# GoekeLab/m6anet

Hardware: AMD Instinct MI355X
Metric: DRACH sites/sec at num_iterations=1000 (higher is better)
Workload: dtype f32

## Files before the change

m6anet_amd/csrc/m6a_api.hip:

```cpp
#include "m6a_ctx.h"

#if !defined(__HIP_DEVICE_COMPILE__)
#ifndef M6A_MT_JUMP_PATH
#error "build with -DM6A_MT_JUMP_PATH=\"<repo>/m6anet_amd/assets/mt19937_jump.bin\" (m6anet_amd/build.py does)"
#endif
asm(".section .rodata\n"
    ".global m6a_mt_jump_blob\n.global m6a_mt_jump_blob_end\n.hidden m6a_mt_jump_blob\n.hidden m6a_mt_jump_blob_end\n.balign 64\n"
    "m6a_mt_jump_blob:\n.incbin \"" M6A_MT_JUMP_PATH "\"\n"
    "m6a_mt_jump_blob_end:\n.byte 0\n.previous\n");
#endif

namespace {

thread_local std::string g_create_error;

std::mutex g_live_mu;
std::vector<m6a_ctx *> g_live;
void join_background_setups()
{
    std::lock_guard<std::mutex> g(g_live_mu);
    for (m6a_ctx *c : g_live)
        if (c->warm.joinable()) c->warm.join();
    g_live.clear();
}
// ... 102 lines not shown
    int64_t start_b = 0;
    for (int64_t b = 0; b < nb; b++) {
        if ((it0 + b + 1) % spb) {
            goff.push_back(std::min((b + 1) * bs, S));
            start_b = b + 1;
        }
    }
    if (start_b < nb) goff.push_back(S);
    return (int64_t)goff.size() - 1;
}

bool base_is_group_start(int64_t base, int64_t bs, int64_t spb)
{
    if (base < 0 || base % bs) return false;
    const int64_t it0 = base / bs;
    return it0 == 0 || (it0 % spb) != 0;
}

int ensure_groups(m6a_ctx *c, int64_t S, int64_t bs, int64_t spb)
{
    const int64_t base = c->job_offset;
    if (c->goff_key.valid && c->goff_key.S == S && c->goff_key.bs == bs && c->goff_key.spb == spb &&
        c->goff_key.base == base) return M6A_OK;
    if (!base_is_group_start(base, bs, spb))
        return fail(c, M6A_EINVAL, "job offset %lld does not start a flush group for batch_size=%lld save_per_batch=%lld",
                    (long long)base, (long long)bs, (long long)spb);
    std::vector<int64_t> g;
    const int64_t G = flush_groups(S, bs, spb, base, g);
    int64_t gmax = 0;
    for (int64_t i = 0; i < G; i++) gmax = std::max(gmax, g[i + 1] - g[i]);
    HIPCHK(c, c->goff.ensure(g.size() * sizeof(int64_t)));
    HIPCHK(c, hipMemcpyAsync(c->goff.p, g.data(), g.size() * sizeof(int64_t), hipMemcpyHostToDevice, c->stream));
    HIPCHK(c, hipStreamSynchronize(c->stream));
    c->goff_key = {S, bs, spb, base, G, gmax, true};
    return M6A_OK;
}

constexpr int kJumpPerRegime = 31, kJumpPolyWords = 312;
constexpr int64_t kXheadWords = 22016;

extern "C" const unsigned char m6a_mt_jump_blob[];
extern "C" const unsigned char m6a_mt_jump_blob_end[];

struct JumpRegime { int64_t G; const uint64_t *polys; };

const JumpRegime *jump_regimes(int *n_out)
// ... 40 lines not shown
    }
    const int n_seg = (int)std::min<int64_t>((len + use->G - 1) / use->G, kJumpPerRegime + 1);
    const size_t poly_bytes = (size_t)kJumpPerRegime * kJumpPolyWords * 8;
    HIPCHK(c, c->mt_scratch.ensure((size_t)kXheadWords * 4 + (size_t)kJumpPerRegime * 1078 * 4 + poly_bytes));
    uint32_t *xhead = (uint32_t *)c->mt_scratch.p, *hist = xhead + kXheadWords;
    uint64_t *d_polys = (uint64_t *)(hist + (size_t)kJumpPerRegime * 1078);
    if (c->mt_polys_G != use->G) {
        HIPCHK(c, hipMemcpyAsync(d_polys, use->polys, poly_bytes, hipMemcpyHostToDevice, c->stream));
        c->mt_polys_G = use->G;
    }
    hipLaunchKernelGGL(mt19937_kernel, dim3(1), dim3(640), 0, c->stream, seed, kXheadWords - 624, raw, (const uint32_t *)nullptr,
                       kXheadWords, xhead, kXheadWords);
    hipLaunchKernelGGL(mt_jump_kernel, dim3(17, (unsigned)(n_seg - 1)), dim3(256), 0, c->stream, (const uint32_t *)xhead,
                       (const uint64_t *)d_polys, hist);
    hipLaunchKernelGGL(mt19937_kernel, dim3((unsigned)n_seg), dim3(640), 0, c->stream, seed, len, raw, (const uint32_t *)hist, use->G,
                       (uint32_t *)nullptr, (int64_t)0);
    HIPCHK(c, hipGetLastError());
    return M6A_OK;
}

int ensure_raw(m6a_ctx *c, uint32_t seed, int64_t len)
{
    if (c->raw_len >= len && c->raw_seed == seed) return M6A_OK;
    if (len > ((int64_t)1 << 31) - 512)
        return fail(c, M6A_ESTREAM, "a flush group would need %lld MT19937 words (cap 2^31); "
                    "reduce batch_size*save_per_batch or num_iterations", (long long)len);
    len = (len + 1023) / 1024 * 1024;
    c->raw_len = 0;
    c->rt.valid = false;
    HIPCHK(c, c->raw.ensure((size_t)len * 4));
    int rc = launch_stream(c, seed, len, (uint32_t *)c->raw.p);
    if (rc) return rc;
    c->raw_seed = seed; c->raw_len = len;
    return M6A_OK;
}

void pairwise_rec(int lo, int n, MeanPlan &p)
{
    if (n <= 128) {
        p.leaf_start.push_back(lo);
        p.merge_after.push_back(0);
        return;
    }
    int n2 = n / 2;
    n2 -= n2 % 8;
    pairwise_rec(lo, n2, p);
// ... 37 lines not shown
    }
    p.reg_ctl.assign((size_t)std::max(1, (T - p.n_rem) / 8), 0u);
    for (int b = 0; b + 1 < L; b++) p.reg_ctl[(size_t)p.leaf_start[b + 1] / 8 - 1] = 1u | ((uint32_t)p.merge_after[b] << 8);
    const int rows = (int)p.row_pass.size();
    p.row_meta.assign((size_t)rows * 4, 0u);
    for (int r = 0; r < rows; r++) {
        uint32_t *m = &p.row_meta[(size_t)r * 4];
        uint64_t live = 0;
        for (int l = 0; l < 64; l++) live |= (uint64_t)(plan_iteration(p, r, l) >= 0) << l;
        m[1] = (uint32_t)live; m[2] = (uint32_t)(live >> 32);
        const int ps = p.row_pass[r];
        if (ps < 0) { m[0] = 1u << 25; continue; }
        if (r + 1 == rows || p.row_pass[r + 1] != ps) {
            const int nl = std::min(8, L - 8 * ps);
            m[0] = (1u << 24) | ((uint32_t)nl << 26) | (ps == P - 1 ? 1u << 30 : 0u);
            for (int bl = 0; bl < nl; bl++) m[3] |= (uint32_t)(p.merge_after[8 * ps + bl] & 15) << (4 * bl);
        }
    }
}

int ensure_mean_plan(m6a_ctx *c, int T)
{
    if (c->plan.T == T && c->plan_dev.p) return M6A_OK;
    build_mean_plan(T, c->plan);
    const MeanPlan &p = c->plan;
    if (p.depth > M6A_MEAN_STACK) return fail(c, M6A_EUNSUPPORTED, "n_iters %d: pairwise-sum tree deeper than %d", T, M6A_MEAN_STACK);
    const size_t b0 = p.leaf_start.size() * 4, b1 = (p.merge_after.size() + 3) / 4 * 4, b2 = std::max<size_t>(p.row_meta.size(), 1) * 4;
    const size_t b3 = p.reg_ctl.size() * 4;
    HIPCHK(c, c->plan_dev.ensure(b0 + b1 + b2 + b3));
    char *d = (char *)c->plan_dev.p;
    HIPCHK(c, hipMemcpyAsync(d, p.leaf_start.data(), b0, hipMemcpyHostToDevice, c->stream));
    HIPCHK(c, hipMemcpyAsync(d + b0, p.merge_after.data(), p.merge_after.size(), hipMemcpyHostToDevice, c->stream));
    if (!p.row_meta.empty())
        HIPCHK(c, hipMemcpyAsync(d + b0 + b1, p.row_meta.data(), p.row_meta.size() * 4, hipMemcpyHostToDevice, c->stream));
    HIPCHK(c, hipMemcpyAsync(d + b0 + b1 + b2, p.reg_ctl.data(), b3, hipMemcpyHostToDevice, c->stream));
    HIPCHK(c, hipStreamSynchronize(c->stream));
    c->plan_off[0] = 0; c->plan_off[1] = b0; c->plan_off[2] = b0 + b1; c->plan_off[3] = b0 + b1 + b2;
    c->tab_key.valid = false;
    return M6A_OK;
}

void plan_args(m6a_ctx *c, PoolArgs &a)
{
    const char *d = (const char *)c->plan_dev.p;
    a.leaf_start = (const int *)(d + c->plan_off[0]);
    a.merge_after = (const uint8_t *)(d + c->plan_off[1]);
// ... 29 lines not shown
    if (n_distinct) *n_distinct = distinct;
    return missing;
}

int ensure_rtab(m6a_ctx *c, uint32_t seed, int T, int K, int64_t gmax, const uint32_t *hist, bool *usable)
{
    *usable = false;
    const int64_t need = stream_need(gmax, T, K);
    int rc = ensure_raw(c, seed, need);
    if (rc) return rc;
    auto &rt = c->rt;
    const int64_t n_blk = c->raw_len / 64;
    if (!(rt.valid && rt.seed == seed && rt.A == (int64_t)T * K && rt.n_blk == n_blk)) {
        rt.valid = false; rt.used = 0;
        for (int n = 0; n <= M6A_RTAB_MAX_N; n++) rt.slot_of_n[n] = -1;
    }
    std::vector<int> todo;
    for (int n = 2; n <= M6A_RTAB_MAX_N; n++)
        if (hist[n] && rt.slot_of_n[n] < 0) todo.push_back(n);
    const int64_t c_stride = n_blk * 64;
    const size_t slot_bytes = (size_t)c_stride * 2 + (size_t)(n_blk + 1) * 4;
    const bool fresh = !rt.valid || rt.n_blk != n_blk;
    const int want = (fresh ? 1 : rt.used) + (int)todo.size();
    if (fresh || want > rt.cap) {
        int new_cap = std::max(want, fresh ? 0 : rt.cap * 2);
        new_cap = std::min(std::max(new_cap, std::max(32, c->rt_presize)), M6A_RTAB_MAX_N + 1);
        size_t free_b = 0, total_b = 0;
        HIPCHK(c, hipMemGetInfo(&free_b, &total_b));
        const size_t held = fresh ? 0 : (size_t)rt.cap * slot_bytes;
        const size_t budget = std::min<size_t>((size_t)16 << 30, (free_b + held) / 2);
        if ((size_t)new_cap * slot_bytes > budget) new_cap = want;
        if ((size_t)new_cap * slot_bytes > budget) return M6A_OK;
        uint16_t *nC = nullptr; uint32_t *nRS = nullptr;
        if (fresh) {
            if (rt.C) (void)hipFree(rt.C);
            if (rt.RS) (void)hipFree(rt.RS);
            rt.C = nullptr; rt.RS = nullptr; rt.cap = 0;
        }
        if (hipMalloc((void **)&nC, (size_t)new_cap * c_stride * 2 + 64) != hipSuccess) { (void)hipGetLastError(); return M6A_OK; }
        if (hipMalloc((void **)&nRS, (size_t)new_cap * (n_blk + 1) * 4) != hipSuccess) { (void)hipGetLastError(); (void)hipFree(nC); return M6A_OK; }
        if (!fresh && rt.used) {
            HIPCHK(c, hipMemcpyAsync(nC, rt.C, (size_t)rt.used * c_stride * 2, hipMemcpyDeviceToDevice, c->stream));
            HIPCHK(c, hipMemcpyAsync(nRS, rt.RS, (size_t)rt.used * (n_blk + 1) * 4, hipMemcpyDeviceToDevice, c->stream));
            HIPCHK(c, hipStreamSynchronize(c->stream));
            c->graveyard.push_back(rt.C); c->graveyard.push_back(rt.RS);
        }
// ... 29 lines not shown
int uniform_slice(m6a_ctx *c, uint32_t seed, int n, int T, int K, int jmax, const uint16_t **C)
{
    *C = nullptr;
    if (n < 2) return M6A_OK;
    std::vector<uint32_t> hist(M6A_HIST_BINS, 0u);
    hist[n] = 1;
    bool usable = false;
    int rc = ensure_rtab(c, seed, T, K, jmax, hist.data(), &usable);
    if (rc) return rc;
    if (!usable) return fail(c, M6A_ENOMEM, "no device memory for the index table of bag size %d", n);
    const int64_t slot = c->rt.slot_of_n[n], A = (int64_t)T * K;
    uint32_t total = 0;
    HIPCHK(c, hipMemcpyAsync(&total, c->rt.RS + slot * (c->rt.n_blk + 1) + c->rt.n_blk, 4, hipMemcpyDeviceToHost, c->stream));
    HIPCHK(c, hipStreamSynchronize(c->stream));
    if ((int64_t)total < A * jmax) return fail(c, M6A_ESTREAM, "MT19937 stream too short for a flush group");
    *C = c->rt.C + slot * c->rt.n_blk * 64;
    return M6A_OK;
}

int ensure_table_reg(m6a_ctx *c, uint32_t seed, int n, int T, int K, int jmax)
{
    auto &k = c->tab_reg_key;
    if (k.valid && k.seed == seed && k.n == n && k.T == T && k.K == K && k.jmax >= jmax) return M6A_OK;
    k.valid = false;
    const size_t per_j = (size_t)(T + 8) * K;
    const size_t bytes = (size_t)jmax * per_j * 2 + 4096;
    HIPCHK(c, c->tab_reg.ensure(bytes));
    HIPCHK(c, hipMemsetAsync(c->tab_reg.p, 0, bytes, c->stream));
    const uint16_t *C = nullptr;
    int rc = uniform_slice(c, seed, n, T, K, jmax, &C);
    if (rc) return rc;
    if (C) {
        const int64_t A = (int64_t)T * K;
        hipLaunchKernelGGL(rtab_to_reg_table_kernel, dim3((unsigned)((A * jmax + 255) / 256)), dim3(256), 0, c->stream,
                           C, A, (int64_t)per_j, jmax, (uint16_t *)c->tab_reg.p);
        HIPCHK(c, hipGetLastError());
    }
    k = {seed, n, T, K, jmax, true};
    return M6A_OK;
}

int ensure_table(m6a_ctx *c, uint32_t seed, int n, int T, int K, int jmax)
{
    int rc = ensure_mean_plan(c, T);
    if (rc) return rc;
    auto &k = c->tab_key;
    if (k.valid && k.seed == seed && k.n == n && k.T == T && k.K == K && k.jmax >= jmax) return M6A_OK;
    k.valid = false;
    const MeanPlan &p = c->plan;
    const int rows = (int)p.row_pass.size();
    c->iter_of.resize((size_t)rows * 64);
    for (int r = 0; r < rows; r++)
        for (int l = 0; l < 64; l++) c->iter_of[(size_t)r * 64 + l] = plan_iteration(p, r, l);
    const size_t words = (size_t)jmax * rows * 5 * 64;
    HIPCHK(c, c->tab.ensure(words * 4 + c->iter_of.size() * 4));
    int *d_iter = (int *)((uint32_t *)c->tab.p + words);
    HIPCHK(c, hipMemcpyAsync(d_iter, c->iter_of.data(), c->iter_of.size() * 4, hipMemcpyHostToDevice, c->stream));
    const uint16_t *C = nullptr;
    rc = uniform_slice(c, seed, n, T, K, jmax, &C);
    if (rc) return rc;
    if (C) {
        hipLaunchKernelGGL(rtab_to_lds_table_kernel, dim3((unsigned)((words + 255) / 256)), dim3(256), 0, c->stream,
                           C, (int64_t)T * K, K, rows, jmax, (const int *)d_iter, (uint32_t *)c->tab.p);
        HIPCHK(c, hipGetLastError());
    } else {
        HIPCHK(c, hipMemsetAsync(c->tab.p, 0, words * 4, c->stream));
    }
    k = {seed, n, T, K, jmax, true};
    return M6A_OK;
}
// ... 33 lines not shown
    HIPCHK(c, hipMemcpyAsync(c->h_minmax, c->d_minmax, 24, hipMemcpyDeviceToHost, c->stream));
    HIPCHK(c, hipMemcpyAsync(c->h_hist, c->d_hist, M6A_HIST_BINS * 4, hipMemcpyDeviceToHost, c->stream));
    HIPCHK(c, hipStreamSynchronize(c->stream));
    c->bag_min = (int64_t)c->h_minmax[0];
    c->bag_max = (int64_t)c->h_minmax[1];
    c->n_reads = (int64_t)c->h_minmax[2];
    return M6A_OK;
}

int bag_stats(m6a_ctx *c, const int64_t *d_off, int64_t S)
{
    const int64_t *h = c->hint_off;
    c->hint_off = nullptr;
    if (!h) return query_bags(c, d_off, S);
    if (h[0] != 0) return fail(c, M6A_EINVAL, "off[0] must be 0");
    host_bag_range(c, h, S);
    if (c->bag_min < 0) return fail(c, M6A_EINVAL, "off[] must be non-decreasing");
    unsigned long long hash = 0;
    for (int i = 0; i < M6A_HIST_BINS; i++) hash += (unsigned long long)c->h_hist[i] * m6a_bin_weight(i);
    hipStream_t st = c->s_prep ? c->s_prep : c->stream;
    if (st != c->stream) {
        HIPCHK(c, hipEventRecord(c->ev_main, c->stream));
        HIPCHK(c, hipStreamWaitEvent(st, c->ev_main, 0));
    }
    HIPCHK(c, hipMemsetAsync(c->d_minmax, 0xff, 8, st));
    HIPCHK(c, hipMemsetAsync(c->d_minmax + 1, 0, 16, st));
    HIPCHK(c, hipMemsetAsync(c->d_hist, 0, M6A_HIST_BINS * 4, st));
    hipLaunchKernelGGL(bag_minmax_kernel, dim3((unsigned)std::min<int64_t>((S + 255) / 256, 512)), dim3(256), 0,
                       st, d_off, S, c->d_minmax, c->d_hist);
    hipLaunchKernelGGL(bag_verify_kernel, dim3(1), dim3(256), 0, st, c->d_minmax, c->d_hist, (unsigned long long)c->bag_min,
                       (unsigned long long)c->bag_max, (unsigned long long)c->n_reads, hash, c->d_err);
    HIPCHK(c, hipGetLastError());
    c->side_work = true;
    return M6A_OK;
}

int launch_encode(m6a_ctx *c, const float *X, const uint8_t *km, const int64_t *off, int64_t S,
                  int64_t R, float *rp)
{
    if (R <= 0 || S <= 0) return M6A_OK;
    EncArgs a;
    a.X = X; a.site_kmers = km; a.off = off; a.wfrag = c->d_wfrag; a.emb = c->d_emb; a.read_prob = rp;
    a.wfrag2 = c->d_wfrag2; a.w1e_tab = c->d_w1e; a.bn = c->d_w1e + M6A_W1E_FLOATS; a.err = c->d_err;
    a.n_sites = S; a.n_reads = R; a.n_tiles = (R + 31) / 32; a.b3 = c->b3;
    a.clk = c->prof.clk_for(0);
    const int64_t max_waves = (int64_t)c->n_cu * 8;
// ... 28 lines not shown
}

int rtab_prepare(m6a_ctx *c, PoolArgs a, int64_t nmax, int64_t gmax, uint32_t seed, bool *use)
{
    *use = false;
    const int T = a.T, K = a.K;
    const int64_t S = a.n_sites;
    const int64_t need = stream_need(gmax, T, K);
    if (nmax > M6A_RTAB_MAX_N || c->scan_driver == 1 || c->scan_driver == 2) {
        if (c->scan_driver == 3)
            return fail(c, M6A_EUNSUPPORTED, "index-table pooling needs every bag <= %d reads (largest: %lld)", M6A_RTAB_MAX_N, (long long)nmax);
        return M6A_OK;
    }
    int distinct = 0;
    const int missing = rtab_missing(c, seed, T, K, need, c->h_hist, &distinct);
    if (c->rt_credit_seed != seed || c->rt_credit_A != (int64_t)T * K) { c->rt_credit_seed = seed; c->rt_credit_A = (int64_t)T * K; c->rt_credit = 0; }
    bool use_rtab = c->scan_driver == 3 || missing == 0 || c->rt_credit + S >= (int64_t)16 * missing;
    if (use_rtab) c->rt_credit = 0; else c->rt_credit += S;
    if (!use_rtab) return M6A_OK;
    int rc = ensure_rtab(c, seed, T, K, gmax, c->h_hist, &use_rtab);
    if (rc) return rc;
    if (!use_rtab) return M6A_OK;
    a.raw = (const uint32_t *)c->raw.p; a.raw_len = c->raw_len;
    HIPCHK(c, c->rt_rank.ensure((size_t)S * 4));
    HIPCHK(c, c->rt_order.ensure((size_t)S * 4));
    HIPCHK(c, c->ctl_dev.ensure(kCtlWords * 4));
    HIPCHK(c, hipEventSynchronize(c->ev_ctl));
    uint32_t *cur = ctl_cursor(c);
    uint32_t run = 0;
    for (int n = M6A_HIST_BINS - 1; n > M6A_RTAB_SMALL_N; n--) { cur[n] = run; run += c->h_hist[n]; }
    for (int x = 0; x < 8; x++)
        for (int n = M6A_RTAB_SMALL_N - ((M6A_RTAB_SMALL_N - x) & 7); n >= 0; n -= 8) { cur[n] = run; run += c->h_hist[n]; }
    std::memcpy(ctl_slot(c), c->rt.slot_of_n, sizeof c->rt.slot_of_n);
    HIPCHK(c, hipMemcpyAsync(c->ctl_dev.p, c->h_ctl, (size_t)(M6A_HIST_BINS + M6A_RTAB_MAX_N + 1) * 4, hipMemcpyHostToDevice, c->stream));
    HIPCHK(c, hipEventRecord(c->ev_ctl, c->stream));
    const RtabUse u = rtab_use(c, nmax);
    const unsigned n_order_blocks = (unsigned)((S + 255) / 256);
    const unsigned n_chain_blocks = (unsigned)std::min<int64_t>((a.n_groups + 3) / 4, (int64_t)c->n_cu * 16);
    hipLaunchKernelGGL(rtab_prep_kernel, dim3(n_order_blocks + n_chain_blocks), dim3(256), 0, c->stream, a, u,
                       (uint32_t *)c->ctl_dev.p, (uint32_t *)c->rt_order.p, n_order_blocks);
    HIPCHK(c, hipGetLastError());
    *use = true;
    return M6A_OK;
}

int launch_pool(m6a_ctx *c, const float *rp, const int64_t *off, int64_t S, int T, int K, float thr,
// ... 103 lines not shown
        c->pool_variant = by_group ? "scan-group" : "scan-site";
        prof_begin(c, 1);
        if (by_group) {
            const unsigned blocks = (unsigned)std::min<int64_t>((a.n_groups + 3) / 4, wave_slots / 4);
            if (K == 20) hipLaunchKernelGGL(pool_scan_group_kernel<20>, dim3(blocks), dim3(256), lds, c->stream, a);
            else hipLaunchKernelGGL(pool_scan_group_kernel<0>, dim3(blocks), dim3(256), lds, c->stream, a);
        } else {
            hipLaunchKernelGGL(pool_scan_start_kernel, dim3((unsigned)std::min<int64_t>((a.n_groups + 3) / 4, (int64_t)c->n_cu * 8)),
                               dim3(256), 0, c->stream, a);
            const unsigned blocks = (unsigned)std::min<int64_t>((S + 3) / 4, wave_slots / 4);
            if (K == 20) hipLaunchKernelGGL(pool_scan_site_kernel<20>, dim3(blocks), dim3(256), lds, c->stream, a);
            else hipLaunchKernelGGL(pool_scan_site_kernel<0>, dim3(blocks), dim3(256), lds, c->stream, a);
        }
        prof_end(c, 1);
    }
    HIPCHK(c, hipGetLastError());
    return M6A_OK;
}

int pool_setup_aside(m6a_ctx *c, const int64_t *off, int64_t S, int T, int K, uint32_t seed, int64_t bs, int64_t spb)
{
    c->prep.ready = false;
    if (S <= 0 || !c->s_prep) return M6A_OK;
    HIPCHK(c, hipStreamWaitEvent(c->s_prep, c->ev_main, 0));
    hipStream_t main_stream = c->stream;
    c->stream = c->s_prep;
    const int rc = launch_pool(c, nullptr, off, S, T, K, 0.0f, seed, bs, spb, nullptr, nullptr, true);
    c->stream = main_stream;
    if (rc) { c->prep.ready = false; return rc; }
    HIPCHK(c, hipEventRecord(c->ev_prep, c->s_prep));
    HIPCHK(c, hipStreamWaitEvent(c->stream, c->ev_prep, 0));
    return M6A_OK;
}

template <int>
static inline void bag_range_loop(const int64_t *off, int64_t S, int64_t *mn_out, int64_t *mx_out)
{
    int64_t mn = INT64_MAX, mx = 0;
    for (int64_t s = 0; s < S; s++) {
        const int64_t n = off[s + 1] - off[s];
        mn = n < mn ? n : mn;
        mx = n > mx ? n : mx;
    }
    *mn_out = mn; *mx_out = mx;
}
__attribute__((target("avx2"))) static void bag_range_avx2(const int64_t *off, int64_t S, int64_t *mn, int64_t *mx) { bag_range_loop<1>(off, S, mn, mx); }
static void bag_range_base(const int64_t *off, int64_t S, int64_t *mn, int64_t *mx) { bag_range_loop<0>(off, S, mn, mx); }

void host_bag_range(m6a_ctx *c, const int64_t *off, int64_t S)
{
    int64_t mn = INT64_MAX, mx = 0;
    static const bool avx2 = __builtin_cpu_supports("avx2");
    (avx2 ? bag_range_avx2 : bag_range_base)(off, S, &mn, &mx);
    auto bin = [](int64_t n) { return n < 0 ? 0 : n > M6A_RTAB_MAX_N ? M6A_RTAB_MAX_N + 1 : n; };
// ... 388 lines not shown
                     (float *)c->sSite.p, (double *)c->sMod.p);
    if (rc) return rc;
    HIPCHK(c, hipMemcpyAsync(site, c->sSite.p, (size_t)S * 4, hipMemcpyDeviceToHost, c->stream));
    HIPCHK(c, hipMemcpyAsync(mod, c->sMod.p, (size_t)S * 8, hipMemcpyDeviceToHost, c->stream));
    return sync_and_check(c);
}

int m6a_infer(m6a_ctx *c, const float *X, const uint8_t *km, const int64_t *off, int64_t S, int T, int K,
              float thr, uint32_t seed, int rng_mode, int64_t bs, int64_t spb, float *rp, float *site, double *mod)
{
    settle(c);
    HintScope hint_scope(c);
    if (c && c->job.open) return job_busy(c);
    int rc = check_pool_args(c, S, T, K, rng_mode, bs, spb);
    if (rc) return rc;
    if (S == 0) return M6A_OK;
    if (!X || !km || !off || !site || !mod) return fail(c, M6A_EINVAL, "null pointer argument");
    HIPCHK(c, hipSetDevice(c->device));
    const bool dev = is_device_ptr(X);
    if (dev != is_device_ptr(km) || dev != is_device_ptr(off) || dev != is_device_ptr(site) ||
        dev != is_device_ptr(mod) || (rp && dev != is_device_ptr(rp)))
        return fail(c, M6A_EINVAL, "all data pointers must be host pointers or all device pointers");
    if (dev) {
        rc = bag_stats(c, off, S);
        if (rc) return rc;
        const int64_t R = c->n_reads;
        float *p = rp;
        if (!p) { HIPCHK(c, c->rp_scratch.ensure((size_t)std::max<int64_t>(R, 1) * 4)); p = (float *)c->rp_scratch.p; }
        HIPCHK(c, hipEventRecord(c->ev_main, c->stream));
        rc = launch_encode(c, X, km, off, S, R, p);
        if (rc) return rc;
        rc = pool_setup_aside(c, off, S, T, K, seed, bs, spb);
        if (rc) return rc;
        return launch_pool(c, p, off, S, T, K, thr, seed, bs, spb, site, mod);
    }
    if (off[0] != 0) return fail(c, M6A_EINVAL, "off[0] must be 0");
    for (int64_t s = 0; s < S; s++) if (off[s + 1] < off[s]) return fail(c, M6A_EINVAL, "off[] must be non-decreasing");
    const int64_t R = off[S];
    HIPCHK(c, c->sSite.ensure((size_t)S * 4));
    HIPCHK(c, c->sMod.ensure((size_t)S * 8));
    host_bag_range(c, off, S);
    Prefault pf_rp, pf_out;
    if (rp) pf_rp.start(rp, (size_t)R * 4, 2);
    pf_out.start(mod, (size_t)S * 8, 1);
    rc = staged_encode(c, X, km, off, S, R, rp);
    if (rc) return rc;
    rc = launch_pool(c, (const float *)c->sP.p, (const int64_t *)c->sOff.p, S, T, K, thr, seed, bs, spb,
                     (float *)c->sSite.p, (double *)c->sMod.p);
    if (rc) return rc;
    return staged_outputs(c, S, site, mod);
}

// ... 169 lines not shown
```

m6anet_amd/csrc/m6a_ctx.h:

```cpp
#pragma once
#include <hip/hip_runtime.h>
#include <dlfcn.h>
#include <sys/mman.h>

#include <algorithm>
#include <atomic>
#include <cmath>
#include <cstdarg>
#include <cstdio>
#include <cstdlib>
#include <cstring>
#include <condition_variable>
#include <functional>
#include <memory>
#include <mutex>
#include <new>
#include <string>
#include <thread>
#include <vector>

#include "m6a.h"
#include "m6a_kernels.h"
#include "m6a_host_cpus.h"

// ... 160 lines not shown
    uint32_t raw_seed = 0; int64_t raw_len = 0;
    struct { uint32_t seed; int n, T, K, jmax; bool valid; } tab_key = {0, 0, 0, 0, 0, false}, tab_reg_key = {0, 0, 0, 0, 0, false};
    int table_variant = 0;
    struct { int64_t S, bs, spb, base, G, gmax; bool valid; } goff_key = {0, 0, 0, 0, 0, 0, false};
    int64_t job_offset = 0;
    int64_t bag_min = 0, bag_max = 0, n_reads = 0;
    int enc_variant = 0;
    const char *enc_variant_used = "none";
    const char *enc_kernel_used = "none";
    int scan_driver = 0;
    int *d_err = nullptr;
    unsigned long long *d_minmax = nullptr;
    unsigned long long *h_minmax = nullptr;
    int *h_err = nullptr;
    uint32_t *h_hist = nullptr, *d_hist = nullptr;
    std::vector<uint32_t> hist_part;
    uint32_t *h_ctl = nullptr;
    DevBuf ctl_dev, rt_rank, rt_order;
    bool side_work = false;
    const int64_t *hint_off = nullptr;
    hipEvent_t ev_ctl = nullptr;
    hipStream_t s_prep = nullptr;
    hipEvent_t ev_main = nullptr, ev_prep = nullptr;
    struct { bool ready = false, use = false; const int64_t *off = nullptr; int64_t S = 0, bs = 0, spb = 0; int T = 0, K = 0; uint32_t seed = 0; } prep;
    struct {
        bool valid = false; uint32_t seed = 0; int64_t A = 0, n_blk = 0;
        int cap = 0, used = 0;
        uint16_t *C = nullptr; uint32_t *RS = nullptr;
        int32_t slot_of_n[M6A_RTAB_MAX_N + 1];
    } rt;
    DevBuf sX, sK, sOff, sP, sSite, sMod, val_idx, val_y, val_avg, sOffChunk;
    Staging stg;
    std::vector<void *> graveyard;
    int rt_presize = 0;
    uint32_t rt_credit_seed = 0; int64_t rt_credit_A = 0, rt_credit = 0;
    struct Job {
        bool open = false;
        int failed = 0;
        std::string failed_msg;
        int T = 0, K = 0; float thr = 0.f; uint32_t seed = 0; int64_t bs = 1, spb = 1;
        std::vector<int64_t> off;
        int64_t S = 0, R = 0;
        int n_sub = 0; size_t sub_bytes = 0, o_goff = 0, o_km = 0, o_x = 0;
        int64_t cap_sites = 0, cap_reads = 0;
        std::vector<char *> pin;
        std::vector<hipEvent_t> ev_h2d, ev_enc;
// ... 62 lines not shown
```

m6anet_amd/csrc/m6a_kernels.hip:

```cpp
#include <hip/hip_runtime.h>
#include <stdint.h>

#include "m6a_kernels.h"

typedef float f32x16 __attribute__((ext_vector_type(16)));
typedef float f32x2 __attribute__((ext_vector_type(2)));

__device__ __forceinline__ float chain8_sum(float r)
{
    r += __builtin_bit_cast(float, __builtin_amdgcn_update_dpp(0, __builtin_bit_cast(int, r), 0xB1, 0xf, 0xf, false));
    r += __builtin_bit_cast(float, __builtin_amdgcn_update_dpp(0, __builtin_bit_cast(int, r), 0x4E, 0xf, 0xf, false));
    r += __builtin_bit_cast(float, __builtin_amdgcn_update_dpp(0, __builtin_bit_cast(int, r), 0x141, 0xf, 0xf, false));
    return r;
}

__device__ __forceinline__ int wave_sum_i32(int v)
{
#pragma unroll
    for (int m = 1; m < 64; m <<= 1) v += __shfl_xor(v, m, 64);
    return v;
}

#define L2_REGS(m) ((m) == 4 ? 12 : 16)

// ... 87 lines not shown
    const float t1 = c + c_other;
    v[0] = __builtin_fmaf(r[8], w[8], half ? 0.0f : t1);
#pragma unroll
    for (int q = 1; q < 7; q++) v[q] = r[8 + q] * w[8 + q];
    v[7] = half ? 0.0f : k0;
    c = ((v[0] + v[4]) + (v[2] + v[6])) + ((v[1] + v[5]) + (v[3] + v[7]));
    c_other = __shfl_xor(c, 32, 64);
    asm volatile("" : "+v"(c_other));
    return c + c_other;
}

__device__ __forceinline__ int64_t uniform_i64(int64_t v)
{
    return ((int64_t)__builtin_amdgcn_readfirstlane((int)(v >> 32)) << 32) |
           (uint32_t)__builtin_amdgcn_readfirstlane((int)v);
}

__device__ __forceinline__ void wave_lds_fence()
{
    __builtin_amdgcn_fence(__ATOMIC_ACQ_REL, "wavefront");
    __builtin_amdgcn_wave_barrier();
}

struct EncTile {
    float f[8];
    int64_t s_last;
};

__global__ __launch_bounds__(256, 2) void enc_kernel(EncArgs a)
{
    clamp_keeps_nan();
    m6a_clk_stamp(a.clk, 0);
    __shared__ float s_emb[132];
    __shared__ __attribute__((aligned(16))) float s_bn[M6A_BN_FLOATS];
    for (int i = threadIdx.x; i < 132; i += 256) s_emb[i] = a.emb[i];
    for (int i = threadIdx.x; i < M6A_BN_FLOATS; i += 256) s_bn[i] = a.bn[i];
    __syncthreads();

    const int lane = threadIdx.x & 63;
    const int col = lane & 31;
    const int half = lane >> 5;
    const float *bn_half = s_bn + half * 32;
    const int64_t wave = (int64_t)blockIdx.x * 4 + __builtin_amdgcn_readfirstlane((int)(threadIdx.x >> 6));
    const int64_t tile0 = wave * a.tiles_per_wave;
    if (tile0 >= a.n_tiles) return;
    const int64_t tile1 = (tile0 + a.tiles_per_wave < a.n_tiles) ? tile0 + a.tiles_per_wave : a.n_tiles;

    float w1[40], w2[80], w3[16];
#pragma unroll
    for (int i = 0; i < 40; i++) w1[i] = a.wfrag[i * 64 + lane];
#pragma unroll
    for (int i = 0; i < 80; i++) w2[i] = a.wfrag[(40 + i) * 64 + lane];
#pragma unroll
    for (int i = 0; i < 16; i++) w3[i] = a.wfrag[(120 + i) * 64 + lane];

    int64_t s_base;
    {
        const int64_t r = tile0 * 32;
        int64_t lo = 0, hi = a.n_sites;
        while (hi - lo > 1) {
            int64_t mid = (lo + hi) >> 1;
            if (a.off[mid] <= r) lo = mid; else hi = mid;
        }
        s_base = lo;
    }
    const int64_t last_site = a.n_sites - 1;

    auto link0 = [&](int64_t base, int64_t (&o)[3]) {
#pragma unroll
        for (int i = 0; i < 3; i++) {
            const int64_t si = base + 1 + i;
            o[i] = a.off[si <= a.n_sites ? si : a.n_sites];
        }
    };
    auto link1 = [&](int64_t tile, int64_t base, const int64_t (&o)[3], int64_t &s, int (&km)[3], float (&x)[8]) {
        const int64_t r = tile * 32 + col;
        const int64_t rc = r < a.n_reads ? r : a.n_reads - 1;
        s = base + (rc >= o[0] ? 1 : 0) + (rc >= o[1] ? 1 : 0);
        if (__any(rc >= o[2])) {
            s = base;
            while (a.off[s + 1] <= rc) ++s;
        }
        s = s < last_site ? s : last_site;
        const uint8_t *kp = a.site_kmers + s * 3;
        km[0] = kp[0]; km[1] = kp[1]; km[2] = kp[2];
        const float *xp = a.X + rc * 9 + half;
#pragma unroll
        for (int i = 0; i < 4; i++) x[i] = xp[2 * i];
// ... 76 lines not shown
    for (int i = threadIdx.x; i < M6A_BN_FLOATS; i += 256) s_bn[i] = a.bn[i];
    __syncthreads();

    const int lane = threadIdx.x & 63;
    const int col = lane & 31;
    const int half = lane >> 5;
    const float *bn_half = s_bn + half * 32;
    const int wave = (int)blockIdx.x * 4 + __builtin_amdgcn_readfirstlane((int)(threadIdx.x >> 6));
    const int n_tiles = (int)a.n_tiles, tpw = (int)a.tiles_per_wave;
    const int tile0 = wave * tpw;
    if (tile0 >= n_tiles) return;
    const int tile1 = (tile0 + tpw < n_tiles) ? tile0 + tpw : n_tiles;
    const int n_sites = (int)a.n_sites;
    const int last_lim = (int)(a.n_reads - 1 - (int64_t)(n_tiles - 1) * 32);

    float w1[40], w2[80], w3[16];
#pragma unroll
    for (int i = 0; i < 40; i++) w1[i] = a.wfrag[i * 64 + lane];
#pragma unroll
    for (int i = 0; i < 80; i++) w2[i] = a.wfrag[(40 + i) * 64 + lane];
#pragma unroll
    for (int i = 0; i < 16; i++) w3[i] = a.wfrag[(120 + i) * 64 + lane];

    int s_base;
    {
        const int64_t r = (int64_t)tile0 * 32;
        int lo = 0, hi = n_sites;
        while (hi - lo > 1) {
            const int mid = (int)(((int64_t)lo + hi) >> 1);
            if (a.off[mid] <= r) lo = mid; else hi = mid;
        }
        s_base = lo;
    }
    const int last_site = n_sites - 1;

    const __attribute__((address_space(4))) int64_t *off_c = (const __attribute__((address_space(4))) int64_t *)a.off;
    auto link0 = [&](int base, int64_t (&o)[3]) {
#pragma unroll
        for (int i = 0; i < 3; i++) {
            const int si = base + 1 + i;
            o[i] = off_c[si <= n_sites ? si : n_sites];
        }
    };
    const int kq = lane < 18 ? lane : 17;
    const int kq_site = kq / 6, kq_byte = (kq % 6) / 2;
    int too_small = 0;
    auto link1 = [&](int tile, int base, const int64_t (&o)[3], int &rel, int &kid, float (&x)[8]) {
        const int64_t rbase = (int64_t)tile * 32;
        const int lim = tile == n_tiles - 1 ? last_lim : 31;
        const int crel = col < lim ? col : lim;
        const int d0 = (int)o[0] - (int)rbase, d1 = (int)o[1] - (int)rbase, d2 = (int)o[2] - (int)rbase;
        rel = (crel >= d0 ? 1 : 0) + (crel >= d1 ? 1 : 0);
        too_small |= lim >= d2 ? 1 : 0;
        const int room = last_site - base;
        const int ksr = kq_site < room ? kq_site : room;
        kid = (int)(a.site_kmers + (int64_t)base * 3)[__umul24((unsigned)ksr, 3u) + (unsigned)kq_byte];
// ... 92 lines not shown
    if (threadIdx.x < 64) s_w3[(threadIdx.x >> 5) * 16 + (threadIdx.x & 15)] = a.wfrag[(120 + (threadIdx.x & 15)) * 64 + (threadIdx.x & 32)];
    __syncthreads();

    const int lane = threadIdx.x & 63;
    const int col = lane & 31;
    const int half = lane >> 5;
    const float *bn_half = s_bn + half * 32;
    const int wave = (int)blockIdx.x * 4 + __builtin_amdgcn_readfirstlane((int)(threadIdx.x >> 6));
    const int n_tiles = (int)a.n_tiles, tpw = (int)a.tiles_per_wave;
    const int tile0 = wave * tpw;
    if (tile0 >= n_tiles) return;
    const int tile1 = (tile0 + tpw < n_tiles) ? tile0 + tpw : n_tiles;
    const int n_sites = (int)a.n_sites;
    const int last_lim = (int)(a.n_reads - 1 - (int64_t)(n_tiles - 1) * 32);

    float w1x[20], w8[5], w2[80];
#pragma unroll
    for (int i = 0; i < 20; i++) w1x[i] = a.wfrag2[i * 64 + lane];
#pragma unroll
    for (int i = 0; i < 5; i++) w8[i] = a.wfrag2[(20 + i) * 64 + lane];
#pragma unroll
    for (int i = 0; i < 80; i++) w2[i] = a.wfrag[(40 + i) * 64 + lane];

    int s_base;
    {
        const int64_t r = (int64_t)tile0 * 32;
        int lo = 0, hi = n_sites;
        while (hi - lo > 1) {
            const int mid = (int)(((int64_t)lo + hi) >> 1);
            if (a.off[mid] <= r) lo = mid; else hi = mid;
        }
        s_base = lo;
    }
    const int last_site = n_sites - 1;

    const __attribute__((address_space(4))) int64_t *off_c = (const __attribute__((address_space(4))) int64_t *)a.off;
    auto link0 = [&](int base, int64_t (&o)[3]) {
#pragma unroll
        for (int i = 0; i < 3; i++) {
            const int si = base + 1 + i;
            o[i] = off_c[si <= n_sites ? si : n_sites];
        }
    };
    const int kq = lane < 18 ? lane : 17;
    const int kq_site = kq / 6, kq_byte = (kq % 6) / 2;
    int too_small = 0;
    auto link1 = [&](int tile, int base, const int64_t (&o)[3], int &rel, int &kid, float (&x)[5]) {
        const int64_t rbase = (int64_t)tile * 32;
        const int lim = tile == n_tiles - 1 ? last_lim : 31;
        const int crel = col < lim ? col : lim;
        const int d0 = (int)o[0] - (int)rbase, d1 = (int)o[1] - (int)rbase, d2 = (int)o[2] - (int)rbase;
        rel = (crel >= d0 ? 1 : 0) + (crel >= d1 ? 1 : 0);
        too_small |= lim >= d2 ? 1 : 0;
        const int room = last_site - base;
        const int ksr = kq_site < room ? kq_site : room;
        kid = (int)(a.site_kmers + (int64_t)base * 3)[__umul24((unsigned)ksr, 3u) + (unsigned)kq_byte];
// ... 765 lines not shown
```

m6anet_amd/csrc/m6a_pool_rtab.hip:

```cpp
#include "m6a_kernels.h"

namespace {

__device__ __forceinline__ uint32_t pow2_mask_u32(uint32_t rng)
{
    uint32_t mask = rng;
    mask |= mask >> 1; mask |= mask >> 2; mask |= mask >> 4; mask |= mask >> 8; mask |= mask >> 16;
    return mask;
}

__device__ __forceinline__ float chain8_sum_r(float r)
{
    r += __builtin_bit_cast(float, __builtin_amdgcn_update_dpp(0, __builtin_bit_cast(int, r), 0xB1, 0xf, 0xf, false));
    r += __builtin_bit_cast(float, __builtin_amdgcn_update_dpp(0, __builtin_bit_cast(int, r), 0x4E, 0xf, 0xf, false));
    r += __builtin_bit_cast(float, __builtin_amdgcn_update_dpp(0, __builtin_bit_cast(int, r), 0x141, 0xf, 0xf, false));
    return r;
}

__device__ __forceinline__ void wave_fence()
{
    __builtin_amdgcn_fence(__ATOMIC_ACQ_REL, "wavefront");
    __builtin_amdgcn_wave_barrier();
}

// ... 262 lines not shown
                if (b0 + 63 > n_blk) b0 = n_blk >= 63 ? n_blk - 63 : 0;
                const uint32_t idx = b0 + lane;
                const uint32_t v = idx <= n_blk ? rs[idx] : 0xffffffffu;
                const int c = __popcll(__ballot(v <= e));
                if (c == 0) { b0 = b0 > 62 ? b0 - 62 : 0; continue; }
                if (c == 64) { b0 += 62; continue; }
                b2 = b0 + (uint32_t)c - 1;
                rs_b2 = (uint32_t)__builtin_amdgcn_readlane((int)v, c - 1);
                break;
            }
            const uint32_t kth = e - rs_b2;
            if (b2 != w_blk) { w = a.raw[(int64_t)b2 * 64 + lane]; w_blk = b2; }
            const bool ok2 = (w & mask) < n;
            const unsigned long long bal2 = __ballot(ok2);
            const uint32_t rank2 = __builtin_amdgcn_mbcnt_hi((uint32_t)(bal2 >> 32), __builtin_amdgcn_mbcnt_lo((uint32_t)bal2, 0));
            const unsigned long long hit = __ballot(ok2 && rank2 == kth);
            p = (uint32_t)uni((int)(b2 * 64 + (uint32_t)__builtin_ctzll(hit) + 1));
        }
    }
}

__device__ __forceinline__ void rtab_order_part(const int64_t *off, int64_t n_sites, uint32_t *cursor, uint32_t *order, unsigned block)
{
    __shared__ uint32_t s_cnt[M6A_HIST_BINS], s_base[M6A_HIST_BINS];
    for (int i = threadIdx.x; i < M6A_HIST_BINS; i += 256) s_cnt[i] = 0;
    __syncthreads();
    const int64_t s = (int64_t)block * 256 + threadIdx.x;
    int64_t n = 0;
    uint32_t mine = 0;
    if (s < n_sites) {
        n = off[s + 1] - off[s];
        n = n < 0 ? 0 : n > M6A_RTAB_MAX_N ? M6A_RTAB_MAX_N + 1 : n;
        mine = atomicAdd(&s_cnt[n], 1u);
    }
    __syncthreads();
    if (s < n_sites && mine == 0) s_base[n] = atomicAdd(&cursor[n], s_cnt[n]);
    __syncthreads();
    if (s < n_sites) order[s_base[n] + mine] = (uint32_t)s;
}

__global__ __launch_bounds__(256) void rtab_prep_kernel(PoolArgs a, RtabUse u, uint32_t *cursor, uint32_t *order, unsigned n_order_blocks)
{
    if (blockIdx.x < n_order_blocks) {
        rtab_order_part(a.off, a.n_sites, cursor, order, blockIdx.x);
    } else {
        rtab_chain_part(a, u, blockIdx.x - n_order_blocks, gridDim.x - n_order_blocks);
    }
}

#define RTAB_BAG_LDS ((16 + M6A_MEAN_STACK) * 4)

template <int B>
__device__ __forceinline__ uint32_t byte_times4(uint32_t w, uint32_t two)
{
    uint32_t r;
    if (B == 0) asm("v_lshlrev_b32_sdwa %0, %1, %2 dst_sel:DWORD dst_unused:UNUSED_PAD src0_sel:DWORD src1_sel:BYTE_0" : "=v"(r) : "v"(two), "v"(w));
    else if (B == 1) asm("v_lshlrev_b32_sdwa %0, %1, %2 dst_sel:DWORD dst_unused:UNUSED_PAD src0_sel:DWORD src1_sel:BYTE_1" : "=v"(r) : "v"(two), "v"(w));
    else if (B == 2) asm("v_lshlrev_b32_sdwa %0, %1, %2 dst_sel:DWORD dst_unused:UNUSED_PAD src0_sel:DWORD src1_sel:BYTE_2" : "=v"(r) : "v"(two), "v"(w));
    else asm("v_lshlrev_b32_sdwa %0, %1, %2 dst_sel:DWORD dst_unused:UNUSED_PAD src0_sel:DWORD src1_sel:BYTE_3" : "=v"(r) : "v"(two), "v"(w));
    return r;
}
// ... 171 lines not shown
```

Before: 386.6 million.

## Skip redundant cross-stream waits, use wave-parallel site search, trim LDS in order pass

```diff
diff --git a/m6anet_amd/csrc/m6a_api.hip b/m6anet_amd/csrc/m6a_api.hip
--- a/m6anet_amd/csrc/m6a_api.hip
+++ b/m6anet_amd/csrc/m6a_api.hip
@@ -148,6 +148,7 @@
     const int64_t base = c->job_offset;
     if (c->goff_key.valid && c->goff_key.S == S && c->goff_key.bs == bs && c->goff_key.spb == spb &&
         c->goff_key.base == base) return M6A_OK;
+    c->setup_enq = true;
     if (!base_is_group_start(base, bs, spb))
         return fail(c, M6A_EINVAL, "job offset %lld does not start a flush group for batch_size=%lld save_per_batch=%lld",
                     (long long)base, (long long)bs, (long long)spb);
@@ -234,6 +235,7 @@
 int ensure_raw(m6a_ctx *c, uint32_t seed, int64_t len)
 {
     if (c->raw_len >= len && c->raw_seed == seed) return M6A_OK;
+    c->setup_enq = true;
     if (len > ((int64_t)1 << 31) - 512)
         return fail(c, M6A_ESTREAM, "a flush group would need %lld MT19937 words (cap 2^31); "
                     "reduce batch_size*save_per_batch or num_iterations", (long long)len);
@@ -317,6 +319,7 @@
 int ensure_mean_plan(m6a_ctx *c, int T)
 {
     if (c->plan.T == T && c->plan_dev.p) return M6A_OK;
+    c->setup_enq = true;
     build_mean_plan(T, c->plan);
     const MeanPlan &p = c->plan;
     if (p.depth > M6A_MEAN_STACK) return fail(c, M6A_EUNSUPPORTED, "n_iters %d: pairwise-sum tree deeper than %d", T, M6A_MEAN_STACK);
@@ -392,6 +395,7 @@
     const size_t slot_bytes = (size_t)c_stride * 2 + (size_t)(n_blk + 1) * 4;
     const bool fresh = !rt.valid || rt.n_blk != n_blk;
     const int want = (fresh ? 1 : rt.used) + (int)todo.size();
+    if (fresh || want > rt.cap || !todo.empty()) c->setup_enq = true;
     if (fresh || want > rt.cap) {
         int new_cap = std::max(want, fresh ? 0 : rt.cap * 2);
         new_cap = std::min(std::max(new_cap, std::max(32, c->rt_presize)), M6A_RTAB_MAX_N + 1);
@@ -467,6 +471,7 @@
 {
     auto &k = c->tab_reg_key;
     if (k.valid && k.seed == seed && k.n == n && k.T == T && k.K == K && k.jmax >= jmax) return M6A_OK;
+    c->setup_enq = true;
     k.valid = false;
     const size_t per_j = (size_t)(T + 8) * K;
     const size_t bytes = (size_t)jmax * per_j * 2 + 4096;
@@ -491,6 +496,7 @@
     if (rc) return rc;
     auto &k = c->tab_key;
     if (k.valid && k.seed == seed && k.n == n && k.T == T && k.K == K && k.jmax >= jmax) return M6A_OK;
+    c->setup_enq = true;
     k.valid = false;
     const MeanPlan &p = c->plan;
     const int rows = (int)p.row_pass.size();
@@ -570,6 +576,7 @@
     if (st != c->stream) {
         HIPCHK(c, hipEventRecord(c->ev_main, c->stream));
         HIPCHK(c, hipStreamWaitEvent(st, c->ev_main, 0));
+        c->ev_main_here = true;
     }
     HIPCHK(c, hipMemsetAsync(c->d_minmax, 0xff, 8, st));
     HIPCHK(c, hipMemsetAsync(c->d_minmax + 1, 0, 16, st));
@@ -644,6 +651,7 @@
     if (rc) return rc;
     if (!use_rtab) return M6A_OK;
     a.raw = (const uint32_t *)c->raw.p; a.raw_len = c->raw_len;
+    c->setup_enq = true;
     HIPCHK(c, c->rt_rank.ensure((size_t)S * 4));
     HIPCHK(c, c->rt_order.ensure((size_t)S * 4));
     HIPCHK(c, c->ctl_dev.ensure(kCtlWords * 4));
@@ -793,14 +801,18 @@
 {
     c->prep.ready = false;
     if (S <= 0 || !c->s_prep) return M6A_OK;
-    HIPCHK(c, hipStreamWaitEvent(c->s_prep, c->ev_main, 0));
+    if (!c->ev_main_here) HIPCHK(c, hipStreamWaitEvent(c->s_prep, c->ev_main, 0));
+    c->ev_main_here = false;
     hipStream_t main_stream = c->stream;
     c->stream = c->s_prep;
+    c->setup_enq = false;
     const int rc = launch_pool(c, nullptr, off, S, T, K, 0.0f, seed, bs, spb, nullptr, nullptr, true);
     c->stream = main_stream;
     if (rc) { c->prep.ready = false; return rc; }
-    HIPCHK(c, hipEventRecord(c->ev_prep, c->s_prep));
-    HIPCHK(c, hipStreamWaitEvent(c->stream, c->ev_prep, 0));
+    if (c->setup_enq) {
+        HIPCHK(c, hipEventRecord(c->ev_prep, c->s_prep));
+        HIPCHK(c, hipStreamWaitEvent(c->stream, c->ev_prep, 0));
+    }
     return M6A_OK;
 }
 
@@ -1235,12 +1247,13 @@
         dev != is_device_ptr(mod) || (rp && dev != is_device_ptr(rp)))
         return fail(c, M6A_EINVAL, "all data pointers must be host pointers or all device pointers");
     if (dev) {
+        c->ev_main_here = false;
         rc = bag_stats(c, off, S);
         if (rc) return rc;
         const int64_t R = c->n_reads;
         float *p = rp;
         if (!p) { HIPCHK(c, c->rp_scratch.ensure((size_t)std::max<int64_t>(R, 1) * 4)); p = (float *)c->rp_scratch.p; }
-        HIPCHK(c, hipEventRecord(c->ev_main, c->stream));
+        if (!c->ev_main_here) HIPCHK(c, hipEventRecord(c->ev_main, c->stream));
         rc = launch_encode(c, X, km, off, S, R, p);
         if (rc) return rc;
         rc = pool_setup_aside(c, off, S, T, K, seed, bs, spb);
diff --git a/m6anet_amd/csrc/m6a_ctx.h b/m6anet_amd/csrc/m6a_ctx.h
--- a/m6anet_amd/csrc/m6a_ctx.h
+++ b/m6anet_amd/csrc/m6a_ctx.h
@@ -206,6 +206,8 @@
     hipEvent_t ev_ctl = nullptr;
     hipStream_t s_prep = nullptr;
     hipEvent_t ev_main = nullptr, ev_prep = nullptr;
+    bool ev_main_here = false;
+    bool setup_enq = false;
     struct { bool ready = false, use = false; const int64_t *off = nullptr; int64_t S = 0, bs = 0, spb = 0; int T = 0, K = 0; uint32_t seed = 0; } prep;
     struct {
         bool valid = false; uint32_t seed = 0; int64_t A = 0, n_blk = 0;
diff --git a/m6anet_amd/csrc/m6a_kernels.hip b/m6anet_amd/csrc/m6a_kernels.hip
--- a/m6anet_amd/csrc/m6a_kernels.hip
+++ b/m6anet_amd/csrc/m6a_kernels.hip
@@ -133,6 +133,21 @@
     __builtin_amdgcn_wave_barrier();
 }
 
+template <typename I> __device__ __forceinline__ I wave_first_site(const int64_t *off, I n_sites, int64_t r, int lane)
+{
+    int64_t lo = 0, hi = n_sites;
+    while (hi - lo > 1) {
+        const int64_t step = (hi - lo + 63) >> 6;
+        const int64_t p = lo + (int64_t)(lane + 1) * step;
+        const bool le = p < hi && off[p < hi ? p : hi] <= r;
+        const int64_t n_le = __popcll(__ballot(le));
+        const int64_t nlo = lo + n_le * step, nhi = nlo + step;
+        lo = nlo;
+        hi = nhi < hi ? nhi : hi;
+    }
+    return (I)lo;
+}
+
 struct EncTile {
     float f[8];
     int64_t s_last;
@@ -165,16 +180,7 @@
 #pragma unroll
     for (int i = 0; i < 16; i++) w3[i] = a.wfrag[(120 + i) * 64 + lane];
 
-    int64_t s_base;
-    {
-        const int64_t r = tile0 * 32;
-        int64_t lo = 0, hi = a.n_sites;
-        while (hi - lo > 1) {
-            int64_t mid = (lo + hi) >> 1;
-            if (a.off[mid] <= r) lo = mid; else hi = mid;
-        }
-        s_base = lo;
-    }
+    int64_t s_base = wave_first_site<int64_t>(a.off, a.n_sites, tile0 * 32, lane);
     const int64_t last_site = a.n_sites - 1;
 
     auto link0 = [&](int64_t base, int64_t (&o)[3]) {
@@ -297,16 +303,7 @@
 #pragma unroll
     for (int i = 0; i < 16; i++) w3[i] = a.wfrag[(120 + i) * 64 + lane];
 
-    int s_base;
-    {
-        const int64_t r = (int64_t)tile0 * 32;
-        int lo = 0, hi = n_sites;
-        while (hi - lo > 1) {
-            const int mid = (int)(((int64_t)lo + hi) >> 1);
-            if (a.off[mid] <= r) lo = mid; else hi = mid;
-        }
-        s_base = lo;
-    }
+    int s_base = wave_first_site<int>(a.off, n_sites, (int64_t)tile0 * 32, lane);
     const int last_site = n_sites - 1;
 
     const __attribute__((address_space(4))) int64_t *off_c = (const __attribute__((address_space(4))) int64_t *)a.off;
@@ -445,16 +442,7 @@
 #pragma unroll
     for (int i = 0; i < 80; i++) w2[i] = a.wfrag[(40 + i) * 64 + lane];
 
-    int s_base;
-    {
-        const int64_t r = (int64_t)tile0 * 32;
-        int lo = 0, hi = n_sites;
-        while (hi - lo > 1) {
-            const int mid = (int)(((int64_t)lo + hi) >> 1);
-            if (a.off[mid] <= r) lo = mid; else hi = mid;
-        }
-        s_base = lo;
-    }
+    int s_base = wave_first_site<int>(a.off, n_sites, (int64_t)tile0 * 32, lane);
     const int last_site = n_sites - 1;
 
     const __attribute__((address_space(4))) int64_t *off_c = (const __attribute__((address_space(4))) int64_t *)a.off;
diff --git a/m6anet_amd/csrc/m6a_pool_rtab.hip b/m6anet_amd/csrc/m6a_pool_rtab.hip
--- a/m6anet_amd/csrc/m6a_pool_rtab.hip
+++ b/m6anet_amd/csrc/m6a_pool_rtab.hip
@@ -308,7 +308,7 @@
 
 __device__ __forceinline__ void rtab_order_part(const int64_t *off, int64_t n_sites, uint32_t *cursor, uint32_t *order, unsigned block)
 {
-    __shared__ uint32_t s_cnt[M6A_HIST_BINS], s_base[M6A_HIST_BINS];
+    __shared__ uint32_t s_cnt[M6A_HIST_BINS];
     for (int i = threadIdx.x; i < M6A_HIST_BINS; i += 256) s_cnt[i] = 0;
     __syncthreads();
     const int64_t s = (int64_t)block * 256 + threadIdx.x;
@@ -320,9 +320,9 @@
         mine = atomicAdd(&s_cnt[n], 1u);
     }
     __syncthreads();
-    if (s < n_sites && mine == 0) s_base[n] = atomicAdd(&cursor[n], s_cnt[n]);
+    if (s < n_sites && mine == 0) s_cnt[n] = atomicAdd(&cursor[n], s_cnt[n]);
     __syncthreads();
-    if (s < n_sites) order[s_base[n] + mine] = (uint32_t)s;
+    if (s < n_sites) order[s_cnt[n] + mine] = (uint32_t)s;
 }
 
 __global__ __launch_bounds__(256) void rtab_prep_kernel(PoolArgs a, RtabUse u, uint32_t *cursor, uint32_t *order, unsigned n_order_blocks)
```

Measured after the change: 387.3 million (median of 5 runs). Within noise of the previous version (+0.2%).
